# Nicholaswogan/clima

Hardware: AMD Instinct MI355X
Metric: radiate() calls/sec (higher is better)
Workload: dtype f64; 1 GPU; ModernEarth column, one Radtran%radiate call: nz=200, nw=1000 (600 IR + 600 solar bins), 8 g-points, 8 zenith angles, nk=5; config 2 of BASELINE.json; parallelism=1 GPU

## Files before the change

clima_amd/csrc/kernels.hip:

```cpp
#include "radtran_dev.h"
#include <algorithm>
#include <cstring>
#include <mutex>
#include <set>
#include <utility>

namespace clima {

static bool ensure_max_lds(const void *fn, int bytes = 160 * 1024) {
  static std::mutex mu;
  static std::set<std::pair<int, const void *>> done;
  int dev = 0;
  if (hipGetDevice(&dev) != hipSuccess) return false;
  std::lock_guard<std::mutex> lk(mu);
  if (done.count({dev, fn})) return true;
  if (hipFuncSetAttribute(fn, hipFuncAttributeMaxDynamicSharedMemorySize, bytes) != hipSuccess) return false;
  done.insert({dev, fn});
  return true;
}
static int device_cus() {
  static std::mutex mu;
  static int cus[64] = {0};
  int dev = 0;
  if (hipGetDevice(&dev) != hipSuccess || dev < 0 || dev >= 64) return 256;
// ... 246 lines not shown
}

constexpr int PREP_AXIS_MAX = 1024;
constexpr int PREP_ZERO_BLOCKS = 32;

__device__ __forceinline__ ColumnDev column_at(const ColumnDev &c0, const BatchStrides &bs, const int cb) {
  ColumnDev c = c0;
  const size_t oc = (size_t)cb * bs.col, op = (size_t)cb * bs.prep;
  c.T += oc; c.P += oc; c.dz += oc; c.dens += oc; c.pdens += oc; c.radii += oc; c.T_surface += oc;
  c.meta += 2 * oc;
  c.log10P += op; c.cols += op; c.foreign_col += op; c.absw += op; c.q += op;
  c.ix += 2 * op;
  return c;
}

__global__ __launch_bounds__(256) void k_prep(PrepParams p) {
  __shared__ double s_axis[PREP_AXIS_MAX];
  const int nz = p.nz;
  const int cb = blockIdx.y;
  const ColumnDev c = column_at(p.col, p.bs, cb);
  const int *src = c.meta + 1 + nz;
  if (blockIdx.x == 0) {
    for (int j = threadIdx.x; j < nz; j += blockDim.x) {
      const double Pj = c.P[j], dzj = c.dz[j];
      double fc = 0.0;
      for (int i0 = 0; i0 < p.nsp; i0 += 8) {
        double d[8];
#pragma unroll
        for (int k = 0; k < 8; k++) d[k] = c.dens[min(i0 + k, p.nsp - 1) * nz + j];
#pragma unroll
        for (int k = 0; k < 8; k++) {
          const int i = i0 + k;
          if (i < p.nsp) {
            const double col = d[k] * dzj;
            c.cols[i * nz + j] = col;
            if (p.has_cont && i != p.LH2O) fc = fc + col;
          }
        }
      }
      c.log10P[j] = log10(Pj);
      c.foreign_col[j] = fc;
    }
    return;
  }
  if ((int)blockIdx.x > p.nslots + p.nabs) {
    const int zb = (int)blockIdx.x - (p.nslots + p.nabs + 1);
    const int arr = zb / PREP_ZERO_BLOCKS, part = zb - arr * PREP_ZERO_BLOCKS;
    double *dst = p.zero_ptr[arr] + (size_t)cb * p.bs.res;
    const size_t n = p.zero_count[arr];
    for (size_t i = (size_t)part * blockDim.x + threadIdx.x; i < n; i += (size_t)PREP_ZERO_BLOCKS * blockDim.x) dst[i] = 0.0;
    return;
  }
  if ((int)blockIdx.x > p.nslots) {
    const int e = (int)blockIdx.x - p.nslots - 1;
    const int a = p.abs_a[e], b = p.abs_b[e], kind = p.abs_kind[e];
    for (int j = threadIdx.x; j < nz; j += blockDim.x) {
      double w;
      if (kind == ABS_CIA) w = c.dens[a * nz + j] * c.dens[b * nz + j] * c.dz[j];
      else if (kind == ABS_COLUMN) w = c.dens[a * nz + j] * c.dz[j];
      else if (kind == ABS_H2O_SELF) w = c.dens[a * nz + j] * (c.dens[a * nz + j] * c.dz[j]);
      else if (kind == ABS_ZERO) w = 0.0;
      else {
        double fc = 0.0;
        for (int i = 0; i < p.nsp; i++)
          if (i != p.LH2O) fc = fc + c.dens[i * nz + j] * c.dz[j];
        w = c.dens[a * nz + j] * fc;
      }
      c.absw[e * nz + j] = w;
    }
    return;
  }
  const int s = blockIdx.x - 1;
  const SlotDev &sl = p.slots[s];
  const bool in_lds = sl.n <= PREP_AXIS_MAX;
  const double *in = sl.source <= 0 ? c.P : sl.source == 1 ? c.T : c.radii + (size_t)(sl.source - 2) * nz;
  const int j0 = threadIdx.x;
  int js0 = 0;
  double x0 = 0.0;
  if (j0 < nz) { js0 = sl.source < 0 ? j0 : src[j0]; x0 = in[j0]; }
  if (in_lds)
    for (int i = threadIdx.x; i < sl.n; i += blockDim.x) s_axis[i] = sl.axis[i];
  __syncthreads();
  const double *axis = in_lds ? s_axis : sl.axis;
  for (int j = threadIdx.x; j < nz; j += blockDim.x) {
    const int js = j == j0 ? js0 : (sl.source < 0 ? j : src[j]);
    const double xin = (j == j0 && js == j) ? x0 : in[js];
    double x;
    if (sl.source < 0) x = log10(xin * 1.0e6);
    else if (sl.source == 0) x = log10(xin);
    else x = xin;
    if (sl.flag_clamp && (x < sl.lo || x > sl.hi)) atomicMax(c.err_flag, p.call_id);
    x = fmin(fmax(x, sl.lo), sl.hi);
    const int i = bracket(axis, sl.n, x);
    c.ix[s * nz + j] = i;
    c.q[s * nz + j] = (x - axis[i]) / (axis[i + 1] - axis[i]);
  }
}

void launch_prep(const PrepParams &p, hipStream_t s) {
  hipLaunchKernelGGL(k_prep, dim3(1 + p.nslots + p.nabs + p.nzero * PREP_ZERO_BLOCKS, p.ncol > 0 ? p.ncol : 1), dim3(256), 0, s, p);
}


__device__ __forceinline__ double lerp1(const double *f, int i, double q) {
  const double p1 = 1.0 - q;
  return p1 * f[i] + q * f[i + 1];
}

constexpr int OP_THREADS = 256;
constexpr int HWREG_HW_ID_WAVE_ID = (3 << 11) | (0 << 6) | 4;

template <bool COHERENT>
// ... 2569 lines not shown
  hipLaunchKernelGGL(k_integrate_partial_b, dim3(p.nchunk, 2, ncol), dim3(256), 0, s, p);
  hipLaunchKernelGGL(k_integrate_final_b, dim3(ncol), dim3(256), 0, s, p);
}

int integrate_chunks(int nbins) { return nbins <= 0 ? 1 : (nbins + INT_CHUNK - 1) / INT_CHUNK; }

#ifndef CLIMA_INT_LV
#define CLIMA_INT_LV 16
#endif
#ifndef CLIMA_INT_CG
#define CLIMA_INT_CG 32
#endif
constexpr int INT_LV = CLIMA_INT_LV;
constexpr int INT_CG = CLIMA_INT_CG;

__global__ __launch_bounds__(INT_LV * INT_CG) void k_integrate_one(IntegrateParams p) {
  extern __shared__ __align__(16) double s_int[];
  const int a = blockIdx.y;
  const bool sol = a >= 2;
  const int nl = p.nz + 1;
  const int lv = threadIdx.x % INT_LV, cg = threadIdx.x / INT_LV;
  const int i = blockIdx.x * INT_LV + lv;
  if (p.timeout_out && a == 0 && blockIdx.x == 0 && blockIdx.z == 0 && threadIdx.x == 0) {
    const int t = *p.timeout_flag;
    *p.timeout_out = (t == p.id_opr ? 1.0 : 0.0) + (t == p.id_sol ? 1024.0 : 0.0);
  }
  if (p.host_out && a == 0 && blockIdx.x == 0 && blockIdx.z == 0 && threadIdx.x < 2)
    reinterpret_cast<int *>(p.host_out + 5 * nl)[threadIdx.x] = p.err_words[threadIdx.x];
  if (sol && !p.do_solar) {
    if (p.flux_part && cg == 0 && i < nl) p.flux_n[a * nl + i] = p.flux_part[a * nl + i];
    if (p.host_out && cg == 0 && i < nl) p.host_out[a * nl + i] = p.flux_n[a * nl + i];
    return;
  }
  const int cb = blockIdx.z;
  const double *src = (a == 0 ? p.ir_fup_a : a == 1 ? p.ir_fdn_a : a == 2 ? p.sol_fup_a : p.sol_fdn_a) + (size_t)cb * p.bs.res;
  double *const flux_n = p.flux_n + (size_t)cb * p.bs.flux;
  const double *freq = sol ? p.sol_freq : p.ir_freq;
  const int lo = sol ? p.sol_lo : p.ir_lo, cnt = sol ? p.sol_n : p.ir_n;
  double *s_df = s_int;
  double *s_part = s_int + (size_t)p.nchunk * INT_CHUNK;
  double v[INT_CHUNK];
  {
    const int l0 = lo + cg * INT_CHUNK;
#pragma unroll
    for (int k = 0; k < INT_CHUNK; k++)
      v[k] = (cg < p.nchunk && i < nl && l0 + k < lo + cnt) ? src[(size_t)(l0 + k) * nl + i] : 0.0;
  }
  for (int k = threadIdx.x; k < p.nchunk * INT_CHUNK; k += blockDim.x)
    s_df[k] = k < cnt ? freq[lo + k] - freq[lo + k + 1] : 0.0;
// ... 9 lines not shown
#pragma unroll
    for (int k = 0; k < INT_CHUNK; k++)
      if (l0 + k < lo + cnt) acc = __builtin_fma(v[k], s_df[ch * INT_CHUNK + k], acc);
    s_part[ch * INT_LV + lv] = acc;
  }
  __syncthreads();
  if (cg == 0 && i < nl) {
    double acc = 0.0;
    for (int k = 0; k < p.nchunk; k++) acc = acc + s_part[k * INT_LV + lv];
    flux_n[a * nl + i] = acc;
    if (p.flux_part) p.flux_part[a * nl + i] = acc;
    if (p.host_out) p.host_out[a * nl + i] = acc;
  }
}

bool integrate_one_launch(const IntegrateParams &p) {
  return sizeof(double) * (size_t)p.nchunk * (INT_CHUNK + INT_LV) <= 64 * 1024;
}

void launch_integrate(const IntegrateParams &p, hipStream_t s) {
  const int nl = p.nz + 1;
  const size_t lds = sizeof(double) * (size_t)p.nchunk * (INT_CHUNK + INT_LV);
  if (lds <= 64 * 1024) {
    hipLaunchKernelGGL(k_integrate_one, dim3((nl + INT_LV - 1) / INT_LV, 4, p.ncol > 0 ? p.ncol : 1), dim3(INT_LV * INT_CG), lds, s, p);
    return;
  }
  hipLaunchKernelGGL(k_integrate_partial, dim3(p.nchunk, 4), dim3(256), 0, s, p);
  hipLaunchKernelGGL(k_integrate_final, dim3(1), dim3(1024), 0, s, p);
}

__global__ __launch_bounds__(256) void k_w0_from_scat(const double *tau, const double *scat, double *w0, int nw, int ng, int nz) {
  const size_t n = (size_t)nw * ng * nz;
// ... 188 lines not shown
```

clima_amd/csrc/radtran_api.hip:

```cpp
#include "../../include/clima_radtran_hip.h"
#include "radtran_dev.h"

#include <rccl/rccl.h>
#include <sys/stat.h>
#include <unistd.h>
#include <ctime>

#include <algorithm>
#include <cmath>
#include <cstdio>
#include <cstdlib>
#include <chrono>
#include <cstring>
#include <functional>
#include <set>
#include <string>
#include <utility>
#include <limits>
#include <vector>

using namespace clima;

namespace {

// ... 189 lines not shown
  DevBuf<double> d_cols_arena, d_flux_arena;
  DevBuf<double> d_prep_arena, d_opr_arena, d_res_arena;
  int batch_cols_in_flight = 64;
  BatchRun dev_batch;
  DevBuf<int> d_batch_nsrc;
  std::vector<int> batch_nsrc;
  hipEvent_t ev_producer = nullptr;
  bool batch_shared = true;
  int rebin_mode = 1;
  long coop_items = 34816;
  bool fused = true;
  bool generic_opacity = false;
  bool ts_block_mode = false;
  int ts_ncols_env = 0;
  DevBuf<int> d_done;
  int profile = 0;
  long timer_calls = 0;
  int profile_stride = 1;
  struct Ev { hipEvent_t a, b; int id; };
  std::vector<Ev> pending;
  std::vector<hipEvent_t> pool;
  double k_ms[4] = {0, 0, 0, 0};
  int k_n[4] = {0, 0, 0, 0};

  ~Radtran() {
    for (auto *x : k) delete x;
    for (auto *x : cia) delete x;
    for (auto *x : ray) delete x;
    for (auto *x : pxs) delete x;
    for (auto *x : part) delete x;
// ... 481 lines not shown
  in.rebin_mode = r->rebin_mode; in.cust_on = r->cust_on; in.compute_opacity = compute_opacity;
  in.all_pairs = compute_opacity && b.all_pairs_exact;
  in.fused = r->fused; in.allow_fused = allow_fused; in.generic_opacity = r->generic_opacity;
  in.ts_block_mode = r->ts_block_mode; in.ts_ncols_env = r->ts_ncols_env; in.coop_items = r->coop_items;
  in.no_half = sw_no_half(); in.allow_paired = sw_paired(); in.w0_from_scat = sw_w0_scat();
  return in;
}

void ensure_w0(Radtran *r) {
  if (r->w0_valid) return;
  launch_w0_from_scat(r->d_tau.p, r->d_scat.p, r->d_w0.p, r->nw, r->ng, r->nz, r->stream);
  HIPCHK(hipGetLastError());
  r->w0_valid = true;
}

void enqueue_radiate(Radtran *r, const CallBufs &b, bool compute_solar, bool compute_opacity, bool allow_fused = true) {
  r->timer_calls++;
  upload_fields(r);
  const bool resident = b.kind == CALL_RESIDENT, chunk = b.kind == CALL_ARENA_CHUNK;
  const ColumnDev col = column_dev(r, b);
  TwoStreamParams ts = make_twostream_params(r, b, col, compute_solar);
  const LaunchPlan plan = plan_radiate(plan_input(r, b, compute_solar, compute_opacity, allow_fused));
  bool fused_done = false;
  if (compute_opacity) {
    const int call_id = ++r->call_id;
    const PrepParams pp = make_prep_params(r, b, col, call_id, plan.prep_clears ? &ts : nullptr);
    { KernelTimer t(r, 0); launch_prep(pp, r->stream); HIPCHK(hipGetLastError()); t.stop(); }

    OpacityParams op = make_opacity_params(r, b, col, plan.write_w0);
    if (plan.fused.form != TS_NONE) {
      FusedParams fp;
      std::memset(&fp, 0, sizeof(fp));
      fp.ncol = b.ncol; fp.bs = b.bs;
      fp.call_id = call_id; fp.max_spins = r->fused_max_spins;
      fp.done = b.done; fp.timeout_flag = r->d_err.p + 1;
      KernelTimer t(r, 1);
      fused_done = launch_fused(op, ts, fp, plan.fused, r->stream);
      HIPCHK(hipGetLastError());
      t.stop();
      if (!fused_done) op = make_opacity_params(r, b, col, true);
    }
    if (chunk && !fused_done) throw HipFail{"internal: a one-launch batch needs the fused grid"};
    if (!fused_done) {
      KernelTimer t(r, 1);
      const bool ok = launch_opacity(op, plan, r->stream);
      HIPCHK(hipGetLastError());
      if (!ok)
        throw HipFail{"k-distributions with " + std::to_string(r->ng) + " g-points are not supported (1..32)"};
      t.stop();
    }
    r->opr_valid = true;
    if (!chunk) r->w0_valid = op.write_w0 != 0;
    if (resident) r->opr_upload_id = r->upload_id;
  } else if (!chunk) {
    ensure_w0(r);
  }
  r->last_cs = compute_solar;
  if (compute_solar) r->solar_id = r->call_id;

  if (!fused_done) {
    KernelTimer t(r, 2);
    bool ok = launch_twostream_w(ts, plan.ts, r->stream);
    if (!ok) { HIPCHK(hipGetLastError()); ok = launch_twostream(ts, plan.block, r->stream); }
    HIPCHK(hipGetLastError());
    if (!ok)
      throw HipFail{"nz*ngauss = " + std::to_string(r->nz * r->ng) + " exceeds what the two-stream kernels can stage"};
    t.stop();
  }

  const bool reduce = r->comm && resident;
  const IntegrateParams ip = make_integrate_params(r, b, compute_solar, reduce);
  r->small_in_host = ip.host_out != nullptr;
  { KernelTimer t(r, 3); launch_integrate(ip, r->stream); HIPCHK(hipGetLastError()); t.stop(); }
  if (reduce) {
    NCCLCHK(ncclAllReduce(r->d_small.p, r->d_small.p, 4 * ((size_t)r->nz + 1) + 1, ncclDouble, ncclSum, r->comm, r->stream));
    r->comm_reduces++;
  }
  r->small_valid = false;
}

bool recover_fused_timeout(Radtran *r);
void settle_device_batch(Radtran *r);

void fetch_small(Radtran *r) {
  settle_device_batch(r);
  if (r->small_valid) return;
  const int nl = r->nz + 1;
  for (int pass = 0; pass < 2; pass++) {
    if (!r->small_in_host)
      HIPCHK(hipMemcpyAsync(r->h_small, r->d_small.p, sizeof(double) * (5 * nl + 1), hipMemcpyDeviceToHost, r->stream));
    HIPCHK(hipStreamSynchronize(r->stream));
    resolve_events(r);
    if (r->comm) r->comm_status = r->h_small[4 * nl];
    if (!r->column_loaded || !recover_fused_timeout(r)) break;
  }
  f_total_row(r->h_small, nl);
  r->small_valid = true;
// ... 6 lines not shown
  if (dim_T != r->nz) { set_err(err, "\"T\" has the wrong input dimension."); return false; }
  if (dim_P != r->nz) { set_err(err, "\"P\" has the wrong input dimension."); return false; }
  if (d1 != r->nz || d2 != r->nsp) { set_err(err, "\"densities\" has the wrong input dimension."); return false; }
  if (dim_dz != r->nz) { set_err(err, "\"dz\" has the wrong input dimension."); return false; }
  if (has_p && radii) {
    if (p1 != r->nz || p2 != r->np) { set_err(err, "\"pdensities\" has the wrong input dimension."); return false; }
    if (r1 != r->nz || r2 != r->np) { set_err(err, "\"radii\" has the wrong input dimension."); return false; }
  }
  return true;
}

void do_upload(Radtran *r, double T_surface, const double *T, const double *P, const double *dens,
               const double *dz, const double *pdens, const double *radii) {
  const int nz = r->nz;
  double *h = r->h_col;
  settle_device_batch(r);
  if (r->upload_pending) { HIPCHK(hipEventSynchronize(r->ev_upload)); r->upload_pending = false; }
  r->nsrc = pack_column(r, h, T_surface, T, P, dz, dens, pdens, radii);
  r->column_has_particles = (pdens && radii);
  r->upload_id++;
  const int *meta = reinterpret_cast<const int *>(h + r->meta_ofs);
  bool all = (nz % 2 == 0) && r->nsrc * 2 == nz;
  for (int m = 0; m < r->nsrc && all; m++) all = (meta[1 + m] & SRC_EXACT) != 0;
  r->all_pairs_exact = all;
  {
    static const bool kcopy = [] { const char *e = getenv("CLIMA_HIP_COPY_KERNEL"); return !(e && e[0] == '0'); }();
    if (kcopy && r->h_col_dev) launch_copy(r->d_col.p, r->h_col_dev, r->col_count, r->stream);
    else HIPCHK(hipMemcpyAsync(r->d_col.p, h, sizeof(double) * r->col_count, hipMemcpyHostToDevice, r->stream));
  }
  HIPCHK(hipEventRecord(r->ev_upload, r->stream));
  r->upload_pending = true;
// ... 114 lines not shown
}
bool settle_batch(Radtran *r, const BatchRun &b) {
  wait_error_words(r);
  if (r->h_errflag[1] >= b.first_call) {
    r->fused_fallbacks++;
    if (b.one_launch && !b.rows) fetch_batch_nsrc(r, b.n);
    enqueue_batch(r, b, false);
    wait_error_words(r);
    r->opr_valid = true;
  }
  r->checked_timeout = r->checked_id = r->call_id;
  invalidate_small(r);
  return *r->h_errflag >= b.first_call;
}
void settle_device_batch(Radtran *r) {
  if (!r->dev_batch.pending) return;
  r->dev_batch.pending = false;
  if (settle_batch(r, r->dev_batch)) defer_err(r, OPACITY_FAILED_MSG);
}
PackParams make_pack_params(Radtran *r, int n, const double *T_surface, const double *T, const double *P, const double *dens,
                            const double *dz, const double *pdens, const double *radii, double *blocks, int *nsrc) {
  PackParams p;
  std::memset(&p, 0, sizeof(p));
  p.ncol = n; p.nz = r->nz; p.nsp = r->nsp; p.np = r->np;
  p.has_particles = r->np > 0 && pdens && radii;
  p.use_radii = p.has_particles && !r->part.empty();
  p.col_count = r->col_count; p.meta_ofs = r->meta_ofs;
  p.T_surface = T_surface; p.T = T; p.P = P; p.dz = dz; p.dens = dens; p.pdens = pdens; p.radii = radii;
  p.blocks = blocks; p.nsrc = nsrc;
  return p;
// ... 319 lines not shown
  Radtran *r = as_rad(ptr);
  *spins = r ? r->fused_max_spins : 0;
}
void radtran_ir_green_set(void *ptr, const int *mode) {
  Radtran *r = as_rad(ptr);
  if (r) r->ir_green_mode = std::max(0, std::min(2, *mode));
}
void radtran_ir_green_get(void *ptr, int *mode, int *batches) {
  Radtran *r = as_rad(ptr);
  *mode = r ? r->ir_green_mode : 0;
  *batches = r ? (int)std::min<long>(r->ir_green_batches, 2147483647L) : 0;
}
void radtran_fused_fallbacks_get(void *ptr, int *count) {
  Radtran *r = as_rad(ptr);
  *count = r ? r->fused_fallbacks : 0;
}

void radtran_unset_custom_optical_properties(void *ptr) {
  Radtran *r = as_rad(ptr);
  if (r) r->cust_on = false;
}

void radtran_create_end(void *ptr, const int *num_zenith_angles, const double *surface_albedo, char *err) {
  clear_err(err);
  GUARD(r, ptr, err);
  if (r->state != 1) { set_err(err, "radtran_create_end: create_begin has not been called"); return; }
  if (r->k.empty()) { set_err(err, "There are no k-distributions, yet there must be some to compute total opacity."); return; }
  if (r->ir.nw == 0 || r->sol.nw == 0) { set_err(err, "wavelength channels are not set"); return; }
  if (*num_zenith_angles < 1) { set_err(err, "number of zenith angles must be >= 1"); return; }
  TRY
// ... 153 lines not shown
  clear_err(err);
  GUARD(r, ptr, err);
  if (r->state != 2) { set_err(err, "Radtran is not constructed"); return; }
  if (r->np > 0 && (!pdensities || !radii)) { set_err(err, "The model contains particles but \"pdensities\" and \"radii\" are not arguments."); return; }
  TRY
  do_upload(r, *T_surface, T, P, densities, dz, pdensities, radii);
  CATCH(err)
}

void radtran_radiate_resident(void *ptr, const int *compute_solar, const int *compute_opacity, char *err) {
  clear_err(err);
  GUARD(r, ptr, err);
  if (r->state != 2) { set_err(err, "Radtran is not constructed"); return; }
  if (!r->column_loaded) { set_err(err, "no column has been uploaded"); return; }
  TRY
  enqueue_radiate(r, resident_bufs(r), *compute_solar != 0, *compute_opacity != 0);
  CATCH(err)
}

static void ir_batch_general(Radtran *r, const double *d_T, const double *d_Ts, int n, double *d_out, size_t out_arr) {
  const int nz = r->nz, nl = nz + 1, nw_ir = r->ir.nw;
  const int CH = std::min(n, 512);
  const int nchunk = integrate_chunks(r->ir_n);
  const size_t spec = (size_t)nw_ir * nl;
  auto ensure = [](DevBuf<double> &b, size_t count) { if (b.n < count) b.alloc(count); };
  ensure(r->d_bup, spec * CH); ensure(r->d_bdn, spec * CH); ensure(r->d_bpartial, (size_t)CH * 2 * nchunk * nl);
  const CallBufs b = resident_bufs(r);
  TwoStreamParams ts = make_twostream_params(r, b, column_dev(r, b), false);
  ts.ir_fup_a = r->d_bup.p; ts.ir_fdn_a = r->d_bdn.p;
  ts.b_T = nz; ts.b_Ts = 1; ts.b_out = spec;
  PlanIn in = plan_input(r, b, false, false, false);
// ... 670 lines not shown
    if (err && err[0]) return;
    radtran_synchronize(ptr, err);
    us[i] = std::chrono::duration<double, std::micro>(std::chrono::steady_clock::now() - t0).count();
    if (err && err[0]) return;
  }
}

void clima_bench_resident_graph(void *ptr, const int *n, const int *k, double *us, char *err) {
  clear_err(err);
  GUARD(r, ptr, err);
  if (r->state != 2 || !r->column_loaded) { set_err(err, "no column has been uploaded"); return; }
  TRY
  const int one = 1;
  radtran_radiate_resident(ptr, &one, &one, err);
  if (err && err[0]) return;
  HIPCHK(hipStreamSynchronize(r->stream));
  if (r->fields_dirty || r->profile != 0) throw HipFail{"clima_bench_resident_graph: not with stale fields or profiling on"};
  hipGraph_t graph = nullptr;
  hipGraphExec_t exec = nullptr;
  HIPCHK(hipStreamBeginCapture(r->stream, hipStreamCaptureModeThreadLocal));
  try {
    enqueue_radiate(r, resident_bufs(r), true, true);
  } catch (...) {
    hipGraph_t g2 = nullptr;
    (void)hipStreamEndCapture(r->stream, &g2);
    if (g2) (void)hipGraphDestroy(g2);
    (void)hipGetLastError();
    throw;
  }
  HIPCHK(hipStreamEndCapture(r->stream, &graph));
// ... 31 lines not shown
    launch_scale(r->wrk_sol.fup_a.p, r->wrk_sol.fup_a.n, *rad_enhancement, r->stream);
    launch_scale(r->d_flux_n.p + 2 * nl, (size_t)2 * nl, *rad_enhancement, r->stream);
    if (r->shard_world > 1 && r->d_flux_part.p) launch_scale(r->d_flux_part.p + 2 * nl, (size_t)2 * nl, *rad_enhancement, r->stream);
    if (!r->comm) launch_f_total(r->nz, r->d_flux_n.p, r->d_f_total.p, r->stream);
    invalidate_small(r);
    fetch_small(r);
    for (int i = 0; i < nl; i++) r->f_total[i] = r->h_small[4 * nl + i];
  } catch (...) {
  }
}

void radtran_flux_device_ptr(void *ptr, void **dptr, int *count) {
  Radtran *r = as_rad(ptr);
  *dptr = r ? (void *)r->d_flux_n.p : nullptr;
  *count = r ? 4 * (r->nz + 1) : 0;
}

void radtran_set_bin_shard(void *ptr, const int *rank, const int *world, char *err) {
  clear_err(err);
  GUARD(r, ptr, err);
  if (r->state != 2) { set_err(err, "Radtran is not constructed"); return; }
  if (*world < 1 || *rank < 0 || *rank >= *world) { set_err(err, "invalid shard (rank, world)"); return; }
  if (r->comm && r->comm_n > 1 && (*world != r->comm_n || *rank != r->comm_rank)) {
    set_err(err, "the bin shard of a handle with a communicator is (rank, nranks) of the communicator");
    return;
  }
  TRY
  HIPCHK(hipStreamSynchronize(r->stream));
  r->shard_rank = *rank; r->shard_world = *world;
  compute_shard(r);
  for (WrkObj *w : {&r->wrk_ir, &r->wrk_sol}) { w->fup_a.zero(r->stream); w->fdn_a.zero(r->stream); w->amean.zero(r->stream); w->tau_band.zero(r->stream); }
  r->d_flux_n.zero(r->stream);
  if (*world > 1) {
    if (r->d_flux_part.n < (size_t)4 * (r->nz + 1)) r->d_flux_part.alloc((size_t)4 * (r->nz + 1));
    r->d_flux_part.zero(r->stream);
  }
  HIPCHK(hipStreamSynchronize(r->stream));
  CATCH(err)
}


void radtran_set_device(const int *device, char *err) {
// ... 6 lines not shown
  CATCH(err)
}

void radtran_comm_unique_id(char *id, char *err) {
  clear_err(err);
  TRY
  static_assert(sizeof(ncclUniqueId) == CLIMA_COMM_ID_BYTES, "CLIMA_COMM_ID_BYTES is RCCL's NCCL_UNIQUE_ID_BYTES");
  ncclUniqueId u;
  NCCLCHK(ncclGetUniqueId(&u));
  std::memcpy(id, &u, sizeof(u));
  CATCH(err)
}

static void comm_attach(Radtran *r, int nranks, int rank, const char *id) {
  if (r->comm) throw HipFail{"this handle already has a communicator"};
  HIPCHK(hipSetDevice(r->device));
  ncclUniqueId u;
  std::memcpy(&u, id, sizeof(u));
  NCCLCHK(ncclCommInitRank(&r->comm, nranks, u, rank));
  r->comm_n = nranks; r->comm_rank = rank;
}

void radtran_comm_init_rank(void *ptr, const int *nranks, const int *rank, const char *id, char *err) {
  clear_err(err);
  GUARD(r, ptr, err);
  if (r->state != 2) { set_err(err, "Radtran is not constructed"); return; }
  if (*nranks < 1 || *rank < 0 || *rank >= *nranks) { set_err(err, "invalid communicator (rank, nranks)"); return; }
  TRY
  comm_attach(r, *nranks, *rank, id);
  CATCH(err)
// ... 72 lines not shown
  const int zero = 0, one = 1;
  char e[CLIMA_ERR_LEN + 1];
  radtran_set_bin_shard(ptr, &zero, &one, e);
}

void radtran_bin_shard_get(void *ptr, int *op_lo, int *op_n, int *ir_lo, int *ir_n, int *sol_lo, int *sol_n) {
  Radtran *r = as_rad(ptr);
  if (!r) return;
  *op_lo = r->op_lo; *op_n = r->op_n; *ir_lo = r->ir_lo; *ir_n = r->ir_n; *sol_lo = r->sol_lo; *sol_n = r->sol_n;
}

void radtran_finish_reduced(void *ptr, char *err) {
  clear_err(err);
  GUARD(r, ptr, err);
  if (r->state != 2) { set_err(err, "Radtran is not constructed"); return; }
  invalidate_small(r);
}

void radtran_stream_get(void *ptr, void **stream) {
  Radtran *r = as_rad(ptr);
  *stream = r ? (void *)r->stream : nullptr;
}

void radtran_profile_set(void *ptr, const int *enable) {
  Radtran *r = as_rad(ptr);
  if (r) r->profile = (*enable == 2) ? 2 : (*enable != 0 ? 1 : 0);
}
void radtran_profile_stride_set(void *ptr, const int *stride) {
  Radtran *r = as_rad(ptr);
  if (r) r->profile_stride = std::max(1, *stride);
// ... 552 lines not shown
```

clima_amd/csrc/radtran_dev.h:

```cpp
#pragma once

#include <hip/hip_runtime.h>

namespace clima {

constexpr int RB_WIN_LO[8] = {0, 1, 5, 10, 18, 27, 39, 52};
constexpr int RB_WIN_HI[8] = {0, 11, 24, 36, 45, 53, 58, 62};
constexpr int RB_TIGHT_LO[8] = {0, 5, 12, 19, 27, 35, 45, 55};
constexpr int RB_TIGHT_HI[8] = {0, 8, 18, 28, 36, 44, 51, 58};

constexpr int MAX_K = 8;
constexpr int MAX_XS = 16;
constexpr int MAX_PART = 4;
constexpr int MAX_ZEN = 16;
constexpr int MAX_SLOTS = 2 * MAX_K + 2 * MAX_XS + 1 + MAX_PART + 1;

constexpr double PLANK = 6.62607004e-34;
constexpr double C_LIGHT = 299792458.0;
constexpr double K_BOLTZ_SI = 1.380649e-23;
constexpr double PI = 3.14159265358979323846e0;
constexpr double SIGMA_SI = 5.670374419e-8;
constexpr double MAX_W0 = 0.99999;
constexpr double MAX_GT = 0.999999;
constexpr double TAU_MIN = 1.0e-20;
// ... 280 lines not shown
  bool write_w0;
};
LaunchPlan plan_radiate(const PlanIn &in);
int ts_clear_ranges(const TwoStreamParams &p, double *ptr[6], size_t count[6]);

void launch_prep(const PrepParams &p, hipStream_t s);
bool launch_opacity(const OpacityParams &p, const LaunchPlan &pl, hipStream_t s);
bool launch_twostream(TwoStreamParams &p, const TsPlan &t, hipStream_t s);
bool launch_twostream_w(TwoStreamParams &p, const TsPlan &t, hipStream_t s);
bool launch_twostream_ir_batch(TwoStreamParams &p, int ncol, hipStream_t s, int force_nw = 0);
int fused_tiles(const OpacityParams &op);
bool launch_fused(const OpacityParams &op, TwoStreamParams ts, FusedParams fp, const TsPlan &f, hipStream_t s);
bool launch_fused_twostream_only(TwoStreamParams &ts, int slots, const int *meta_nsrc, hipStream_t s, bool half = false, bool paired = false);
void launch_integrate(const IntegrateParams &p, hipStream_t s);
bool integrate_one_launch(const IntegrateParams &p);
void launch_integrate_batch(const BatchIntegrateParams &p, int ncol, hipStream_t s);
int integrate_chunks(int nbins);
void launch_f_total(int nz, const double *flux_n, double *f_total, hipStream_t s);
void launch_scale(double *a, size_t n, double f, hipStream_t s);
void launch_copy(double *dst, const double *src, size_t n, hipStream_t s);
void launch_test_rcp(const double *x, double *y, int n, hipStream_t s);
void launch_test_wscan(const double *a, const double *b, double *out, int nwaves, hipStream_t s);
void launch_w0_from_scat(const double *tau, const double *scat, double *w0, int nw, int ng, int nz, hipStream_t s);
void launch_test_exp(const double *x, double *y, int n, hipStream_t s);
void launch_test_exp_tab(const double *x, double *y, int n, int base10, hipStream_t s);

}
```

clima_amd/lib.py:

```python
import ctypes as C
import os

_HERE = os.path.dirname(os.path.abspath(__file__))
LIB_PATH = os.environ.get("CLIMA_HIP_LIB") or os.path.join(_HERE, "csrc", "libclima_radtran_hip.so")
ERR_LEN = 1024

_dp = C.POINTER(C.c_double)
_ip = C.POINTER(C.c_int)
_bp = C.POINTER(C.c_bool)
_vp = C.c_void_p
_vpp = C.POINTER(C.c_void_p)
_err = C.c_char_p

SIGNATURES = {
    "allocate_radtran": [_vpp],
    "deallocate_radtran": [_vp],
    "radtran_create_begin": [_vp, _ip, _ip, _ip, _ip, _dp, _err],
    "radtran_add_ktable": [_vp, _ip, _ip, _dp, _ip, _dp, _ip, _dp, _dp, _err],
    "radtran_add_xsection": [_vp, _ip, _ip, _ip, _ip, _ip, _dp, _dp, _err],
    "radtran_set_water_continuum": [_vp, _ip, _ip, _dp, _dp, _dp, _err],
    "radtran_add_particle": [_vp, _ip, _ip, _dp, _dp, _dp, _dp, _err],
    "radtran_set_channels": [_vp, _ip, _dp, _ip, _dp, _err],
    "radtran_set_photons_sol": [_vp, _ip, _dp, _err],
    "radtran_create_end": [_vp, _ip, _dp, _err],
    "radtran_radiate_wrapper": [_vp, _dp, _ip, _dp, _ip, _dp, _ip, _ip, _dp, _ip, _dp, _ip, _ip, _ip, _dp, _ip, _ip,
                                _dp, _ip, _ip, _err],
    "radtran_toa_fluxes_wrapper": [_vp, _dp, _ip, _dp, _ip, _dp, _ip, _ip, _dp, _ip, _dp, _ip, _ip, _ip, _dp, _ip, _ip,
                                   _dp, _ip, _ip, _dp, _dp, _err],
    "radtran_apply_radiation_enhancement": [_vp, _dp],
    "radtran_set_custom_optical_properties": [_vp, _ip, _dp, _ip, _dp, _ip, _ip, _dp, _ip, _ip, _dp, _ip, _ip, _dp, _err],
    "radtran_unset_custom_optical_properties": [_vp],
    "radtran_opacities2yaml_wrapper_1": [_vp, _ip, _vpp],
    "radtran_opacities2yaml_wrapper_2": [_vp, _vpp, _ip, _err],
    "radtran_set_names": [_vp, _err, _err, _err],
    "radtran_set_opacity_labels": [_vp, _err, _err, _err, _err],
    "radtran_fused_set": [_vp, _ip],
    "radtran_fused_get": [_vp, _ip],
    "radtran_fused_fallbacks_get": [_vp, _ip],
    "radtran_ir_green_set": [_vp, _ip],
    "radtran_ir_green_get": [_vp, _ip, _ip],
    "radtran_coop_items_set": [_vp, _ip],
    "radtran_coop_items_get": [_vp, _ip],
    "radtran_fused_spins_set": [_vp, _ip],
    "radtran_fused_spins_get": [_vp, _ip],
    "radtran_spectra_get_all": [_vp, _bp, _ip, _ip, _ip, _dp, _dp, _dp, _dp, _dp, _dp, _dp, _err],
    "radtran_spectra_release": [_vp],
    "radtran_create_from_files": [_vp, C.c_char_p, C.c_char_p, _ip, _dp, _ip, C.c_char_p, _err],
    "radtran_load_from_files": [_vp, C.c_char_p, C.c_char_p, _ip, C.c_char_p, _err],
    "clima_test_host_tables_digest": [_vp, C.POINTER(C.c_ulonglong)],
    "radtran_dims_get": [_vp, _ip, _ip, _ip, _ip, _ip],
    "radtran_names_get": [_vp, _ip, C.c_char_p, C.c_char_p],
    "radtran_toa_fluxes_batch": [_vp, _ip, _dp, _dp, _dp, _dp, _dp, _ip, _dp, _dp, _dp, _dp, _dp, _err],
    "radtran_toa_fluxes_batch_device": [_vp, _ip, _vp, _vp, _vp, _vp, _vp, _ip, _vp, _vp, _vp, _vp, _vp, _vp, _err],
# ... 110 lines not shown
```

clima_amd/radtran.py:

```python
import ctypes as C
import os

import numpy as np

from . import lib as _lib

_dp = C.POINTER(C.c_double)


class ClimaException(Exception):
    """clima/cython/_clima.pyx: raised with the Fortran `err` text."""


def _d(a):
    return a.ctypes.data_as(_dp)


def _i(v):
    return C.byref(C.c_int(int(v)))


def _f(v):
    return C.byref(C.c_double(float(v)))

# ... 483 lines not shown
    def ir_green(self, mode):
        self._L.radtran_ir_green_set(self._ptr, _i(int(mode)))

    @property
    def ir_green_batches(self):
        m, b = C.c_int(), C.c_int()
        self._L.radtran_ir_green_get(self._ptr, C.byref(m), C.byref(b))
        return b.value

    @property
    def fused_fallbacks(self):
        v = C.c_int()
        self._L.radtran_fused_fallbacks_get(self._ptr, C.byref(v))
        return v.value

    def flux_tensor(self):
        import torch
        ptr, n = self.flux_device_ptr()

        class _Alias:
            __cuda_array_interface__ = {"shape": (n,), "typestr": "<f8", "data": (ptr, False), "version": 2}

        return torch.as_tensor(_Alias(), device="cuda")

    def finish_reduced(self):
        self._L.radtran_finish_reduced(self._ptr, self._err)
        self._check()

    def flux_device_ptr(self):
        p, n = C.c_void_p(), C.c_int()
# ... 119 lines not shown
```

include/clima_radtran_hip.h:

```cpp
#ifndef CLIMA_RADTRAN_HIP_H
#define CLIMA_RADTRAN_HIP_H

#ifndef __cplusplus
#include <stdbool.h>
#endif

#ifdef __cplusplus
extern "C" {
#endif

#define CLIMA_ERR_LEN 1024

#define CLIMA_XS_CIA 0
#define CLIMA_XS_RAYLEIGH 1
#define CLIMA_XS_ABSORPTION 2
#define CLIMA_XS_PHOTOLYSIS 3


void allocate_radtran(void **ptr);
void deallocate_radtran(void *ptr);

void radtran_create_begin(void *ptr, const int *nz, const int *nsp, const int *np,
                          const int *nw, const double *wavl, char *err);
void radtran_add_ktable(void *ptr, const int *sp_ind, const int *ngauss,
// ... 97 lines not shown
void radtran_dims_get(void *ptr, int *nz, int *nsp, int *np, int *nw, int *ngauss);
void radtran_names_get(void *ptr, const int *cap, char *species_names, char *particle_names);
void radtran_spectra_get_all(void *ptr, const bool *do_solar, const int *nlev, const int *nw_ir, const int *nw_sol,
                             double *ir_fup_a, double *ir_fdn_a, double *ir_tau_band,
                             double *sol_fup_a, double *sol_fdn_a, double *sol_amean, double *sol_tau_band, char *err);
void radtran_spectra_release(void *ptr);
void radtran_batch_pin_results_set(void *ptr, const int *flag);
void radtran_batch_pin_results_get(void *ptr, int *flag);
void radtran_coop_items_set(void *ptr, const int *items);
void radtran_coop_items_get(void *ptr, int *items);
void radtran_fused_spins_set(void *ptr, const int *spins);
void radtran_fused_spins_get(void *ptr, int *spins);
void radtran_ir_green_set(void *ptr, const int *mode);
void radtran_ir_green_get(void *ptr, int *mode, int *batches);
void radtran_fused_fallbacks_get(void *ptr, int *count);
void radtran_stream_get(void *ptr, void **stream);
void radtran_profile_set(void *ptr, const int *enable);
void radtran_profile_stride_set(void *ptr, const int *stride);
void radtran_kernel_time_get(void *ptr, const int *kernel_id, double *ms_total, int *launches,
                             char *err);
void radtran_profile_reset(void *ptr);
void radtran_algorithmic_bytes(void *ptr, double *bytes_tables_distinct, double *bytes_in,
                               double *bytes_out, double *bytes_tables_full, char *err);

void radtran_algorithmic_nodes(void *ptr, double *n_pt, double *n_pt_full, double *n_t, double *n_t_full, char *err);

void clima_bench_toa_fluxes(void *ptr, const int *n, const double *T_surface, const int *dim_T, const double *T,
                            const int *dim_P, const double *P, const int *dim1_d, const int *dim2_d,
                            const double *densities, const int *dim_dz, const double *dz, const int *has_particles,
                            const int *dim1_p, const int *dim2_p, const double *pdensities, const int *dim1_r,
// ... 77 lines not shown
```

Measured before the change: 11270 calls/s.

## Defer resident integration and merge it into the next call's prep kernel

```diff
diff --git a/clima_amd/csrc/kernels.hip b/clima_amd/csrc/kernels.hip
--- a/clima_amd/csrc/kernels.hip
+++ b/clima_amd/csrc/kernels.hip
@@ -284,13 +284,12 @@
   return c;
 }
 
-__global__ __launch_bounds__(256) void k_prep(PrepParams p) {
+__device__ __forceinline__ void prep_block(const PrepParams &p, const int bx, const int cb) {
   __shared__ double s_axis[PREP_AXIS_MAX];
   const int nz = p.nz;
-  const int cb = blockIdx.y;
   const ColumnDev c = column_at(p.col, p.bs, cb);
   const int *src = c.meta + 1 + nz;
-  if (blockIdx.x == 0) {
+  if (bx == 0) {
     for (int j = threadIdx.x; j < nz; j += blockDim.x) {
       const double Pj = c.P[j], dzj = c.dz[j];
       double fc = 0.0;
@@ -313,16 +312,16 @@
     }
     return;
   }
-  if ((int)blockIdx.x > p.nslots + p.nabs) {
-    const int zb = (int)blockIdx.x - (p.nslots + p.nabs + 1);
+  if (bx > p.nslots + p.nabs) {
+    const int zb = bx - (p.nslots + p.nabs + 1);
     const int arr = zb / PREP_ZERO_BLOCKS, part = zb - arr * PREP_ZERO_BLOCKS;
     double *dst = p.zero_ptr[arr] + (size_t)cb * p.bs.res;
     const size_t n = p.zero_count[arr];
     for (size_t i = (size_t)part * blockDim.x + threadIdx.x; i < n; i += (size_t)PREP_ZERO_BLOCKS * blockDim.x) dst[i] = 0.0;
     return;
   }
-  if ((int)blockIdx.x > p.nslots) {
-    const int e = (int)blockIdx.x - p.nslots - 1;
+  if (bx > p.nslots) {
+    const int e = bx - p.nslots - 1;
     const int a = p.abs_a[e], b = p.abs_b[e], kind = p.abs_kind[e];
     for (int j = threadIdx.x; j < nz; j += blockDim.x) {
       double w;
@@ -340,7 +339,7 @@
     }
     return;
   }
-  const int s = blockIdx.x - 1;
+  const int s = bx - 1;
   const SlotDev &sl = p.slots[s];
   const bool in_lds = sl.n <= PREP_AXIS_MAX;
   const double *in = sl.source <= 0 ? c.P : sl.source == 1 ? c.T : c.radii + (size_t)(sl.source - 2) * nz;
@@ -366,6 +365,8 @@
     c.q[s * nz + j] = (x - axis[i]) / (axis[i + 1] - axis[i]);
   }
 }
+
+__global__ __launch_bounds__(256) void k_prep(PrepParams p) { prep_block(p, blockIdx.x, blockIdx.y); }
 
 void launch_prep(const PrepParams &p, hipStream_t s) {
   hipLaunchKernelGGL(k_prep, dim3(1 + p.nslots + p.nabs + p.nzero * PREP_ZERO_BLOCKS, p.ncol > 0 ? p.ncol : 1), dim3(256), 0, s, p);
@@ -2965,25 +2966,22 @@
 constexpr int INT_LV = CLIMA_INT_LV;
 constexpr int INT_CG = CLIMA_INT_CG;
 
-__global__ __launch_bounds__(INT_LV * INT_CG) void k_integrate_one(IntegrateParams p) {
-  extern __shared__ __align__(16) double s_int[];
-  const int a = blockIdx.y;
+__device__ __forceinline__ void integrate_block(const IntegrateParams &p, const int bx, const int a, const int cb, double *s_int) {
   const bool sol = a >= 2;
   const int nl = p.nz + 1;
   const int lv = threadIdx.x % INT_LV, cg = threadIdx.x / INT_LV;
-  const int i = blockIdx.x * INT_LV + lv;
-  if (p.timeout_out && a == 0 && blockIdx.x == 0 && blockIdx.z == 0 && threadIdx.x == 0) {
+  const int i = bx * INT_LV + lv;
+  if (p.timeout_out && a == 0 && bx == 0 && cb == 0 && threadIdx.x == 0) {
     const int t = *p.timeout_flag;
     *p.timeout_out = (t == p.id_opr ? 1.0 : 0.0) + (t == p.id_sol ? 1024.0 : 0.0);
   }
-  if (p.host_out && a == 0 && blockIdx.x == 0 && blockIdx.z == 0 && threadIdx.x < 2)
+  if (p.host_out && a == 0 && bx == 0 && cb == 0 && threadIdx.x < 2)
     reinterpret_cast<int *>(p.host_out + 5 * nl)[threadIdx.x] = p.err_words[threadIdx.x];
   if (sol && !p.do_solar) {
     if (p.flux_part && cg == 0 && i < nl) p.flux_n[a * nl + i] = p.flux_part[a * nl + i];
     if (p.host_out && cg == 0 && i < nl) p.host_out[a * nl + i] = p.flux_n[a * nl + i];
     return;
   }
-  const int cb = blockIdx.z;
   const double *src = (a == 0 ? p.ir_fup_a : a == 1 ? p.ir_fdn_a : a == 2 ? p.sol_fup_a : p.sol_fdn_a) + (size_t)cb * p.bs.res;
   double *const flux_n = p.flux_n + (size_t)cb * p.bs.flux;
   const double *freq = sol ? p.sol_freq : p.ir_freq;
@@ -3023,8 +3021,34 @@
   }
 }
 
+__global__ __launch_bounds__(INT_LV * INT_CG) void k_integrate_one(IntegrateParams p) {
+  extern __shared__ __align__(16) double s_int[];
+  integrate_block(p, blockIdx.x, blockIdx.y, blockIdx.z, s_int);
+}
+
+static_assert(sizeof(PrepParams) + sizeof(IntegrateParams) <= 4096, "k_prep_integrate: the two parameter blocks share the 4 KiB kernel-argument segment");
+__global__ __launch_bounds__(INT_LV * INT_CG) void k_prep_integrate(PrepParams pp, IntegrateParams ip) {
+  extern __shared__ __align__(16) double s_int[];
+  const int nlb = (ip.nz + 1 + INT_LV - 1) / INT_LV;
+  const int b = blockIdx.x;
+  if (b < 4 * nlb) integrate_block(ip, b % nlb, b / nlb, 0, s_int);
+  else prep_block(pp, b - 4 * nlb, 0);
+}
+
 bool integrate_one_launch(const IntegrateParams &p) {
   return sizeof(double) * (size_t)p.nchunk * (INT_CHUNK + INT_LV) <= 64 * 1024;
+}
+
+bool prep_integrate_merges(const PrepParams &pp, const IntegrateParams &ip) {
+  const size_t lds = sizeof(double) * ((size_t)ip.nchunk * (INT_CHUNK + INT_LV) + PREP_AXIS_MAX);
+  return pp.ncol <= 1 && ip.ncol <= 1 && pp.nzero == 0 && pp.nz == ip.nz && !ip.host_out && !ip.timeout_out &&
+         integrate_one_launch(ip) && lds <= 48 * 1024;
+}
+
+void launch_prep_integrate(const PrepParams &pp, const IntegrateParams &ip, hipStream_t s) {
+  const int nlb = (ip.nz + 1 + INT_LV - 1) / INT_LV;
+  const size_t lds = sizeof(double) * (size_t)ip.nchunk * (INT_CHUNK + INT_LV);
+  hipLaunchKernelGGL(k_prep_integrate, dim3(4 * nlb + 1 + pp.nslots + pp.nabs), dim3(INT_LV * INT_CG), lds, s, pp, ip);
 }
 
 void launch_integrate(const IntegrateParams &p, hipStream_t s) {
diff --git a/clima_amd/csrc/radtran_api.hip b/clima_amd/csrc/radtran_api.hip
--- a/clima_amd/csrc/radtran_api.hip
+++ b/clima_amd/csrc/radtran_api.hip
@@ -227,6 +227,11 @@
   bool ts_block_mode = false;
   int ts_ncols_env = 0;
   DevBuf<int> d_done;
+  bool defer_integration = true;
+  bool flux_ptr_taken = false;
+  bool int_pending = false;
+  IntegrateParams pending_ip;
+  long merged_integrations = 0, standalone_integrations = 0;
   int profile = 0;
   long timer_calls = 0;
   int profile_stride = 1;
@@ -738,7 +743,35 @@
   r->w0_valid = true;
 }
 
-void enqueue_radiate(Radtran *r, const CallBufs &b, bool compute_solar, bool compute_opacity, bool allow_fused = true) {
+bool defer_allowed(bool switch_on, int shard_world, bool has_comm, int profile, bool capturing, bool flux_ptr_taken) {
+  return switch_on && shard_world == 1 && !has_comm && profile != 1 && !capturing && !flux_ptr_taken;
+}
+bool defer_allowed_but_for_capture(const Radtran *r) {
+  return defer_allowed(r->defer_integration, r->shard_world, r->comm != nullptr, r->profile, false, r->flux_ptr_taken);
+}
+bool stream_capturing(Radtran *r) {
+  hipStreamCaptureStatus st = hipStreamCaptureStatusNone;
+  HIPCHK(hipStreamIsCapturing(r->stream, &st));
+  return st != hipStreamCaptureStatusNone;
+}
+bool defer_eligible(Radtran *r) {
+  return defer_allowed_but_for_capture(r) && !stream_capturing(r);
+}
+bool resolve_pending_integration(Radtran *r, const PrepParams *prep = nullptr) {
+  if (!r->int_pending) return false;
+  r->int_pending = false;
+  if (prep && r->profile != 1 && prep_integrate_merges(*prep, r->pending_ip) && !stream_capturing(r)) {
+    launch_prep_integrate(*prep, r->pending_ip, r->stream);
+    HIPCHK(hipGetLastError());
+    r->merged_integrations++;
+    return true;
+  }
+  { KernelTimer t(r, 3); launch_integrate(r->pending_ip, r->stream); HIPCHK(hipGetLastError()); t.stop(); }
+  r->standalone_integrations++;
+  return false;
+}
+
+void enqueue_radiate(Radtran *r, const CallBufs &b, bool compute_solar, bool compute_opacity, bool allow_fused = true, bool defer = false) {
   r->timer_calls++;
   upload_fields(r);
   const bool resident = b.kind == CALL_RESIDENT, chunk = b.kind == CALL_ARENA_CHUNK;
@@ -749,7 +782,9 @@
   if (compute_opacity) {
     const int call_id = ++r->call_id;
     const PrepParams pp = make_prep_params(r, b, col, call_id, plan.prep_clears ? &ts : nullptr);
-    { KernelTimer t(r, 0); launch_prep(pp, r->stream); HIPCHK(hipGetLastError()); t.stop(); }
+    if (!resolve_pending_integration(r, resident && !plan.prep_clears ? &pp : nullptr)) {
+      KernelTimer t(r, 0); launch_prep(pp, r->stream); HIPCHK(hipGetLastError()); t.stop();
+    }
 
     OpacityParams op = make_opacity_params(r, b, col, plan.write_w0);
     if (plan.fused.form != TS_NONE) {
@@ -776,8 +811,9 @@
     r->opr_valid = true;
     if (!chunk) r->w0_valid = op.write_w0 != 0;
     if (resident) r->opr_upload_id = r->upload_id;
-  } else if (!chunk) {
-    ensure_w0(r);
+  } else {
+    resolve_pending_integration(r);
+    if (!chunk) ensure_w0(r);
   }
   r->last_cs = compute_solar;
   if (compute_solar) r->solar_id = r->call_id;
@@ -795,7 +831,12 @@
   const bool reduce = r->comm && resident;
   const IntegrateParams ip = make_integrate_params(r, b, compute_solar, reduce);
   r->small_in_host = ip.host_out != nullptr;
-  { KernelTimer t(r, 3); launch_integrate(ip, r->stream); HIPCHK(hipGetLastError()); t.stop(); }
+  if (defer && resident && !reduce && !ip.host_out && integrate_one_launch(ip) && defer_eligible(r)) {
+    r->pending_ip = ip;
+    r->int_pending = true;
+  } else {
+    KernelTimer t(r, 3); launch_integrate(ip, r->stream); HIPCHK(hipGetLastError()); t.stop();
+  }
   if (reduce) {
     NCCLCHK(ncclAllReduce(r->d_small.p, r->d_small.p, 4 * ((size_t)r->nz + 1) + 1, ncclDouble, ncclSum, r->comm, r->stream));
     r->comm_reduces++;
@@ -805,6 +846,7 @@
 
 bool recover_fused_timeout(Radtran *r);
 void settle_device_batch(Radtran *r);
+void settle_pending_batch(Radtran *r);
 
 void fetch_small(Radtran *r) {
   settle_device_batch(r);
@@ -841,7 +883,7 @@
                const double *dz, const double *pdens, const double *radii) {
   const int nz = r->nz;
   double *h = r->h_col;
-  settle_device_batch(r);
+  settle_pending_batch(r);
   if (r->upload_pending) { HIPCHK(hipEventSynchronize(r->ev_upload)); r->upload_pending = false; }
   r->nsrc = pack_column(r, h, T_surface, T, P, dz, dens, pdens, radii);
   r->column_has_particles = (pdens && radii);
@@ -986,6 +1028,10 @@
   return *r->h_errflag >= b.first_call;
 }
 void settle_device_batch(Radtran *r) {
+  resolve_pending_integration(r);
+  settle_pending_batch(r);
+}
+void settle_pending_batch(Radtran *r) {
   if (!r->dev_batch.pending) return;
   r->dev_batch.pending = false;
   if (settle_batch(r, r->dev_batch)) defer_err(r, OPACITY_FAILED_MSG);
@@ -1335,6 +1381,23 @@
 void radtran_fused_fallbacks_get(void *ptr, int *count) {
   Radtran *r = as_rad(ptr);
   *count = r ? r->fused_fallbacks : 0;
+}
+void radtran_defer_integration_set(void *ptr, const int *enable) {
+  Radtran *r = as_rad(ptr);
+  if (r) r->defer_integration = (*enable != 0);
+}
+void radtran_defer_integration_get(void *ptr, int *enabled) {
+  Radtran *r = as_rad(ptr);
+  *enabled = (r && r->defer_integration) ? 1 : 0;
+}
+void clima_test_defer_allowed(const int *switch_on, const int *shard_world, const int *has_comm, const int *profile,
+                              const int *capturing, const int *flux_ptr_taken, int *allowed) {
+  *allowed = defer_allowed(*switch_on != 0, *shard_world, *has_comm != 0, *profile, *capturing != 0, *flux_ptr_taken != 0) ? 1 : 0;
+}
+void radtran_merged_integrations_get(void *ptr, int *merged, int *standalone) {
+  Radtran *r = as_rad(ptr);
+  *merged = r ? (int)std::min<long>(r->merged_integrations, 2147483647L) : 0;
+  *standalone = r ? (int)std::min<long>(r->standalone_integrations, 2147483647L) : 0;
 }
 
 void radtran_unset_custom_optical_properties(void *ptr) {
@@ -1518,7 +1581,7 @@
   if (r->state != 2) { set_err(err, "Radtran is not constructed"); return; }
   if (!r->column_loaded) { set_err(err, "no column has been uploaded"); return; }
   TRY
-  enqueue_radiate(r, resident_bufs(r), *compute_solar != 0, *compute_opacity != 0);
+  enqueue_radiate(r, resident_bufs(r), *compute_solar != 0, *compute_opacity != 0, true, true);
   CATCH(err)
 }
 
@@ -2219,6 +2282,7 @@
   const int one = 1;
   radtran_radiate_resident(ptr, &one, &one, err);
   if (err && err[0]) return;
+  settle_device_batch(r);
   HIPCHK(hipStreamSynchronize(r->stream));
   if (r->fields_dirty || r->profile != 0) throw HipFail{"clima_bench_resident_graph: not with stale fields or profiling on"};
   hipGraph_t graph = nullptr;
@@ -2280,6 +2344,9 @@
   Radtran *r = as_rad(ptr);
   *dptr = r ? (void *)r->d_flux_n.p : nullptr;
   *count = r ? 4 * (r->nz + 1) : 0;
+  if (!r) return;
+  r->flux_ptr_taken = true;
+  try { settle_device_batch(r); } catch (const HipFail &f) { defer_err(r, f.msg); }
 }
 
 void radtran_set_bin_shard(void *ptr, const int *rank, const int *world, char *err) {
@@ -2292,6 +2359,7 @@
     return;
   }
   TRY
+  settle_device_batch(r);
   HIPCHK(hipStreamSynchronize(r->stream));
   r->shard_rank = *rank; r->shard_world = *world;
   compute_shard(r);
@@ -2328,6 +2396,7 @@
 
 static void comm_attach(Radtran *r, int nranks, int rank, const char *id) {
   if (r->comm) throw HipFail{"this handle already has a communicator"};
+  settle_device_batch(r);
   HIPCHK(hipSetDevice(r->device));
   ncclUniqueId u;
   std::memcpy(&u, id, sizeof(u));
@@ -2430,6 +2499,9 @@
   clear_err(err);
   GUARD(r, ptr, err);
   if (r->state != 2) { set_err(err, "Radtran is not constructed"); return; }
+  TRY
+  settle_device_batch(r);
+  CATCH(err)
   invalidate_small(r);
 }
 
diff --git a/clima_amd/csrc/radtran_dev.h b/clima_amd/csrc/radtran_dev.h
--- a/clima_amd/csrc/radtran_dev.h
+++ b/clima_amd/csrc/radtran_dev.h
@@ -318,6 +318,8 @@
 bool launch_fused_twostream_only(TwoStreamParams &ts, int slots, const int *meta_nsrc, hipStream_t s, bool half = false, bool paired = false);
 void launch_integrate(const IntegrateParams &p, hipStream_t s);
 bool integrate_one_launch(const IntegrateParams &p);
+bool prep_integrate_merges(const PrepParams &pp, const IntegrateParams &ip);
+void launch_prep_integrate(const PrepParams &pp, const IntegrateParams &ip, hipStream_t s);
 void launch_integrate_batch(const BatchIntegrateParams &p, int ncol, hipStream_t s);
 int integrate_chunks(int nbins);
 void launch_f_total(int nz, const double *flux_n, double *f_total, hipStream_t s);
diff --git a/clima_amd/lib.py b/clima_amd/lib.py
--- a/clima_amd/lib.py
+++ b/clima_amd/lib.py
@@ -37,6 +37,10 @@
     "radtran_fused_set": [_vp, _ip],
     "radtran_fused_get": [_vp, _ip],
     "radtran_fused_fallbacks_get": [_vp, _ip],
+    "radtran_defer_integration_set": [_vp, _ip],
+    "radtran_defer_integration_get": [_vp, _ip],
+    "radtran_merged_integrations_get": [_vp, _ip, _ip],
+    "clima_test_defer_allowed": [_ip, _ip, _ip, _ip, _ip, _ip, _ip],
     "radtran_ir_green_set": [_vp, _ip],
     "radtran_ir_green_get": [_vp, _ip, _ip],
     "radtran_coop_items_set": [_vp, _ip],
diff --git a/clima_amd/radtran.py b/clima_amd/radtran.py
--- a/clima_amd/radtran.py
+++ b/clima_amd/radtran.py
@@ -521,6 +521,22 @@
         self._L.radtran_fused_fallbacks_get(self._ptr, C.byref(v))
         return v.value
 
+    @property
+    def defer_integration(self):
+        v = C.c_int()
+        self._L.radtran_defer_integration_get(self._ptr, C.byref(v))
+        return bool(v.value)
+
+    @defer_integration.setter
+    def defer_integration(self, on):
+        self._L.radtran_defer_integration_set(self._ptr, _i(1 if on else 0))
+
+    @property
+    def merged_integrations(self):
+        m, s = C.c_int(), C.c_int()
+        self._L.radtran_merged_integrations_get(self._ptr, C.byref(m), C.byref(s))
+        return m.value, s.value
+
     def flux_tensor(self):
         import torch
         ptr, n = self.flux_device_ptr()
diff --git a/include/clima_radtran_hip.h b/include/clima_radtran_hip.h
--- a/include/clima_radtran_hip.h
+++ b/include/clima_radtran_hip.h
@@ -135,6 +135,11 @@
 void radtran_ir_green_set(void *ptr, const int *mode);
 void radtran_ir_green_get(void *ptr, int *mode, int *batches);
 void radtran_fused_fallbacks_get(void *ptr, int *count);
+void radtran_defer_integration_set(void *ptr, const int *enable);
+void radtran_defer_integration_get(void *ptr, int *enabled);
+void radtran_merged_integrations_get(void *ptr, int *merged, int *standalone);
+void clima_test_defer_allowed(const int *switch_on, const int *shard_world, const int *has_comm, const int *profile,
+                              const int *capturing, const int *flux_ptr_taken, int *allowed);
 void radtran_stream_get(void *ptr, void **stream);
 void radtran_profile_set(void *ptr, const int *enable);
 void radtran_profile_stride_set(void *ptr, const int *stride);
```

Result: faster. 11760 calls/s (median of 6 runs) (+4.3%).
